# MILAB-IIT-CV/ATDN_vSLAM

Hardware: AMD Instinct MI355X
Metric: frame-pairs/sec, KITTI 1241x376 odometry inference at 1/2/4/8 MI355X (higher is better)
Workload: dtype f32 via 3xf16 split MFMA (fp32 accumulate); 1 GPU; KITTI seq-03-shaped 376x1241 uint8 frames (resident in HBM) resized to 376x1232, GMA flow 12 GRU iters + CLVO head -> 6-DoF trajectory (BASELINE configs[1]); streams_per_gpu=2, gru_iters=12, parallelism=pairs sharded x1, one all-gather of 512-d features, replicated LSTM scan

## Files before the change

atdn_vslam_amd/csrc/attention.hip:

```cpp
#include "attention.h"

#include <type_traits>

#include "conv_mfma.h"
#include "sf.h"

namespace atdn {
namespace {

constexpr float LOG2E = 1.4426950408889634f;

typedef float v4f __attribute__((ext_vector_type(4)));
typedef float f32x4v __attribute__((ext_vector_type(4)));

__device__ __forceinline__ f16x8 ld_frag(const char* p) { return *reinterpret_cast<const f16x8*>(p); }
__device__ __forceinline__ f16x8 ld_frag_nt(const char* p) {
  const v4f t = __builtin_nontemporal_load(reinterpret_cast<const v4f*>(p));
  return __builtin_bit_cast(f16x8, t);
}
__device__ __forceinline__ void st_frag_nt(char* p, f16x8 v) {
  __builtin_nontemporal_store(__builtin_bit_cast(v4f, v), reinterpret_cast<v4f*>(p));
}
__device__ __forceinline__ f32x16 mfma(f16x8 a, f16x8 b, f32x16 c) { return __builtin_amdgcn_mfma_f32_32x32x16_f16(a, b, c, 0, 0, 0); }
typedef __fp16 fp16x4_tr_ __attribute__((__vector_size__(4 * sizeof(__fp16))));
__device__ __forceinline__ f16x4 ld_tr4(const char* p) {
  return __builtin_bit_cast(f16x4, __builtin_amdgcn_ds_read_tr16_b64_v4f16(
                                       (__attribute__((address_space(3))) fp16x4_tr_*)(p)));
}

typedef unsigned int u32x2 __attribute__((ext_vector_type(2)));
typedef _Float16 f16x2 __attribute__((ext_vector_type(2)));
__device__ __forceinline__ void h3_encode(const float* v_in, float gsum, f16x8& hi, u32x2& bytes, bool& clamped) {
  float v[8];
#pragma unroll
  for (int i = 0; i < 8; ++i) v[i] = v_in[i];
  if (__builtin_expect(!(gsum <= 65504.f), 0)) {
    asm volatile("; h3_encode: saturated group");
#pragma unroll
    for (int i = 0; i < 8; ++i) {
      clamped |= !(v[i] <= 65504.f);
      v[i] = fminf(v[i], 65504.f);
    }
  }
  float hf[8];
#pragma unroll
  for (int i = 0; i < 8; ++i) {
    hi[i] = (_Float16)v[i];
    hf[i] = (float)hi[i];
  }
  const float mx = fmaxf(fmaxf(fmaxf(hf[0], hf[1]), fmaxf(hf[2], hf[3])), fmaxf(fmaxf(hf[4], hf[5]), fmaxf(hf[6], hf[7])));
  const unsigned ef = max(__float_as_uint(mx) >> 23, 113u);
  const float inv_unit = __uint_as_float((272u - ef) << 23);
  unsigned w0 = 0, w1 = 0;
#pragma unroll
  for (int i = 0; i < 8; ++i) {
    const float q = __builtin_fmaf(v[i] - hf[i], inv_unit, 128.f);
    if (i < 4) w0 = __builtin_amdgcn_cvt_pk_u8_f32(q, i, w0); else w1 = __builtin_amdgcn_cvt_pk_u8_f32(q, i - 4, w1);
  }
  bytes[0] = w0;
  bytes[1] = w1;
}
__device__ __forceinline__ f16x8 h3_decode_lo(f16x8 hi, u32x2 bytes) {
  typedef unsigned int u32x4 __attribute__((ext_vector_type(4)));
  const u32x4 hb = __builtin_bit_cast(u32x4, hi);
  const unsigned up = max(max(hb[0], hb[1]), max(hb[2], hb[3]));
  const unsigned lw = max(max(hb[0] & 0xFFFFu, hb[1] & 0xFFFFu), max(hb[2] & 0xFFFFu, hb[3] & 0xFFFFu));
  const unsigned e = max(max(up >> 26, lw >> 10), 1u);
  const float unit = __uint_as_float((e + 94u) << 23);
  const float off = -128.f * unit;
  f16x8 lo;
#pragma unroll
  for (int i = 0; i < 8; ++i) {
    const unsigned w = bytes[i >> 2];
    const float q = (float)((w >> (8 * (i & 3))) & 255u);
    float r = __builtin_fmaf(q, unit, off);
    asm("" : "+v"(r));
    lo[i] = (_Float16)r;
  }
  return lo;
}

template <bool STATS, bool FAST>
__global__ __launch_bounds__(256, 2) void qk_softmax_kernel(const float* __restrict__ qk, const AttnGeom g,
                                                           const float* __restrict__ rowmax_in,
                                                           float* __restrict__ rowmax_out, float* __restrict__ P,
                                                           float* __restrict__ rinv) {
  constexpr int KROW = 160;
  constexpr int KT = 64;
  constexpr int CH = KT * KROW;
  constexpr int IMG = 4 * CH;
  constexpr bool FULL = !STATS && !FAST;
  constexpr int RB = STATS ? 4 : 2;
  constexpr int SR = 16 * RB;
  constexpr int BLK = AT_BLK_BYTES;
  __shared__ __attribute__((aligned(16))) char lds[2 * IMG];

  const int tid = threadIdx.x, lane = tid & 63, wave = tid >> 6;
  const int nstrip = STATS ? (g.Npad + SR - 1) / SR : g.RT;
  const int tiles = (nstrip + 3) >> 2;
  const int id = xcd_remap(blockIdx.x, g.B * tiles);
  const int b = id / tiles, tile = id - b * tiles;
  const int strip = tile * 4 + wave;
  const bool strip_ok = strip < nstrip;
  const int n16 = lane & 15, g16 = lane >> 4;
  const char* qkb = reinterpret_cast<const char*>(qk + (long)b * g.N * 256);

  f16x8 qh[RB][4], ql[RB][4];
  int mrow[RB];
#pragma unroll
  for (int rb = 0; rb < RB; ++rb) {
    mrow[rb] = strip * SR + 16 * rb + n16;
    const char* qrow = qkb + (long)min(mrow[rb], g.N - 1) * 1024 + 16 * g16;
#pragma unroll
    for (int c = 0; c < 4; ++c) {
      qh[rb][c] = ld_frag(qrow + c * 128);
      if (FULL) ql[rb][c] = ld_frag(qrow + c * 128 + 64);
    }
  }

  const int lr = tid >> 3, ls = tid & 7;
  v4f kreg[2][4];
  auto fetch = [&](int j) __attribute__((always_inline)) {
#pragma unroll
    for (int i = 0; i < 2; ++i) {
      const int n = min(j * KT + lr + 32 * i, g.N - 1);
      const char* src = qkb + (long)n * 1024 + 512 + 16 * ls;
#pragma unroll
      for (int c = 0; c < 4; ++c) kreg[i][c] = *reinterpret_cast<const v4f*>(src + c * 128);
    }
  };
  auto stash = [&](int buf) __attribute__((always_inline)) {
#pragma unroll
    for (int i = 0; i < 2; ++i)
#pragma unroll
      for (int c = 0; c < 4; ++c)
        *reinterpret_cast<v4f*>(lds + buf * IMG + c * CH + (lr + 32 * i) * KROW + 16 * ls) = kreg[i][c];
  };

  const int NHT = (g.Q + 1) >> 1;
  float run[RB];
  float c0[RB];
#pragma unroll
  for (int rb = 0; rb < RB; ++rb) {
    c0[rb] = 0.f;
    run[rb] = STATS ? -INFINITY : 0.f;
    if (!STATS) c0[rb] = (float)AT_SHIFT - rowmax_in[(long)b * g.Npad + min(mrow[rb], g.Npad - 1)] * LOG2E;
  }
  bool clamped = false;
  char* pdst = reinterpret_cast<char*>(P) + ((long)(b * g.RT + min(strip, g.RT - 1)) * g.Q) * BLK;

  fetch(0);
  stash(0);
  __syncthreads();
  fetch(min(1, NHT - 1));
  for (int j = 0; j < NHT; ++j) {
    const char* img = lds + (j & 1) * IMG + n16 * KROW + 16 * g16;
    f32x4v acc[4][RB];
#pragma unroll
    for (int kb = 0; kb < 4; ++kb)
#pragma unroll
      for (int rb = 0; rb < RB; ++rb)
#pragma unroll
        for (int e = 0; e < 4; ++e) acc[kb][rb][e] = 0.f;
    f16x8 kh[2][4], kl[2][4];
    auto read_keys = [&](int set, int c) __attribute__((always_inline)) {
#pragma unroll
      for (int kb = 0; kb < 4; ++kb) {
        const char* kp = img + c * CH + 16 * kb * KROW;
        kh[set][kb] = ld_frag(kp);
        if (FULL) kl[set][kb] = ld_frag(kp + 64);
      }
    };
    read_keys(0, 0);
#pragma unroll
    for (int c = 0; c < 4; ++c) {
      if (c + 1 < 4) read_keys((c + 1) & 1, c + 1);
      __builtin_amdgcn_sched_barrier(0);
#pragma unroll
      for (int kb = 0; kb < 4; ++kb)
#pragma unroll
        for (int rb = 0; rb < RB; ++rb) {
          f32x4v a = acc[kb][rb];
          if (FULL) {
            a = __builtin_amdgcn_mfma_f32_16x16x32_f16(kl[c & 1][kb], qh[rb][c], a, 0, 0, 0);
            a = __builtin_amdgcn_mfma_f32_16x16x32_f16(kh[c & 1][kb], ql[rb][c], a, 0, 0, 0);
          }
          a = __builtin_amdgcn_mfma_f32_16x16x32_f16(kh[c & 1][kb], qh[rb][c], a, 0, 0, 0);
          acc[kb][rb] = a;
        }
      __builtin_amdgcn_sched_barrier(0);
    }
    stash((j + 1) & 1);
    fetch(min(j + 2, NHT - 1));
    auto epilogue = [&](auto tail_tag) __attribute__((always_inline)) {
      constexpr bool TAIL = decltype(tail_tag)::value;
#pragma unroll
      for (int cq = 0; cq < 2; ++cq) {
        const int key0 = j * KT + 32 * cq + 4 * g16;
        u32x2 bytes2[2] = {{0u, 0u}, {0u, 0u}};
#pragma unroll
        for (int rb = 0; rb < RB; ++rb) {
          if constexpr (STATS) {
#pragma unroll
            for (int i = 0; i < 8; ++i)
              if (!TAIL || key0 + (i & 3) + 16 * (i >> 2) < g.N) run[rb] = fmaxf(run[rb], acc[2 * cq + (i >> 2)][rb][i & 3]);
          } else {
            float v[8];
#pragma unroll
            for (int i = 0; i < 8; ++i) {
              const float x = __builtin_amdgcn_exp2f(fmaf(acc[2 * cq + (i >> 2)][rb][i & 3], LOG2E, c0[rb]));
              v[i] = (!TAIL || key0 + (i & 3) + 16 * (i >> 2) < g.N) ? x : 0.f;
            }
            const float gsum = ((v[0] + v[1]) + (v[2] + v[3])) + ((v[4] + v[5]) + (v[6] + v[7]));
            run[rb] += gsum;
            const int q = 2 * j + cq;
            if (strip_ok && q < g.Q) {
              char* d = pdst + (long)q * BLK;
              f16x8 hi;
              u32x2 bytes;
              h3_encode(v, gsum, hi, bytes, clamped);
              st_frag_nt(d + rb * 1024 + lane * 16, hi);
              bytes2[rb] = bytes;
            }
          }
        }
        if (!STATS && strip_ok && 2 * j + cq < g.Q) {
          typedef unsigned int u32x4s __attribute__((ext_vector_type(4)));
          const u32x4s bb = {bytes2[0][0], bytes2[0][1], bytes2[1][0], bytes2[1][1]};
          __builtin_nontemporal_store(bb, reinterpret_cast<u32x4s*>(pdst + (long)(2 * j + cq) * BLK + 2048 + lane * 16));
        }
      }
    };
    if ((j + 1) * KT > g.N) {
      asm volatile("; qk_softmax: tail tile");
      epilogue(std::true_type{});
    } else {
      epilogue(std::false_type{});
    }
    __syncthreads();
  }
  sf_report(clamped);
#pragma unroll
  for (int rb = 0; rb < RB; ++rb) {
    float r_ = run[rb];
    if (STATS) {
      r_ = fmaxf(r_, __shfl_xor(r_, 16));
      r_ = fmaxf(r_, __shfl_xor(r_, 32));
      if (g16 == 0 && strip_ok && mrow[rb] < g.Npad) rowmax_out[(long)b * g.Npad + mrow[rb]] = r_;
    } else {
      r_ += __shfl_xor(r_, 16);
      r_ += __shfl_xor(r_, 32);
      if (g16 == 0 && strip_ok) rinv[(long)b * g.Npad + mrow[rb]] = (mrow[rb] < g.N && r_ > 0.f) ? 1.0f / r_ : 0.f;
    }
  }
}

#ifdef ATDN_ATTN_STAMP
__device__ unsigned atdn_attn_stamps_dev[1024][2][8];
#define STAMP(k) do { __builtin_amdgcn_sched_barrier(0); asm volatile("s_waitcnt lgkmcnt(0)" ::: "memory"); \
    const unsigned long long t_ = __builtin_amdgcn_s_memtime(); asm volatile("s_waitcnt lgkmcnt(0)" ::: "memory"); \
    seg[k] += (unsigned)(t_ - tlast); tlast = t_; __builtin_amdgcn_sched_barrier(0); } while (0)
#else
#define STAMP(k) do {} while (0)
#endif
template <bool FAST, bool SPLIT = false>
__global__ __launch_bounds__(512, 2) void attn_v3_kernel(const float* __restrict__ P, const float* __restrict__ rinv,
                                                        const AttnGeom g, const float* __restrict__ vT,
                                                        const float* __restrict__ gamma, const float* __restrict__ mf,
                                                        float* __restrict__ out, const long sb, const int ld,
                                                        const int qsplit = 0, float* __restrict__ part = nullptr) {
  (void)vT; (void)gamma;
  constexpr int VROW = 544;
  constexpr int IMG = 32 * VROW;
  constexpr int BLK = AT_BLK_BYTES;
  constexpr int D = 3;
  constexpr int DEC2 = 14;
  __shared__ __attribute__((aligned(16))) char lds[3 * IMG];

  const int tid = threadIdx.x, lane = tid & 63, wave = tid >> 6;
  const bool setA = wave < 4;
  const int tiles = (g.RT + 7) >> 3;
  const int nsplit = SPLIT ? (g.Q + qsplit - 1) / qsplit : 1;
  const int id0 = xcd_remap(blockIdx.x, g.B * tiles * nsplit);
  const int ks = SPLIT ? id0 % nsplit : 0;
  const int id = SPLIT ? id0 / nsplit : id0;
  const int b = id / tiles, tile = id - b * tiles;
  const int strip = tile * 8 + wave;
  const bool strip_ok = strip < g.RT;
  const int n16 = lane & 15, g16 = lane >> 4;
  const int qlo = SPLIT ? ks * qsplit : 0;
  const int Q = SPLIT ? min(qsplit, g.Q - qlo) : g.Q;

  const char* pblk = reinterpret_cast<const char*>(P) + ((long)(b * g.RT + min(strip, g.RT - 1)) * g.Q + qlo) * BLK;
  typedef unsigned int u32x4s __attribute__((ext_vector_type(4)));
  f16x8 ring[D][2];
  u32x4s ringb[D];
  auto loadP = [&](int q, int slot) __attribute__((always_inline)) {
    const char* p = pblk + (long)min(q, Q - 1) * BLK;
#pragma unroll
    for (int rb = 0; rb < 2; ++rb) ring[slot][rb] = ld_frag_nt(p + rb * 1024 + lane * 16);
    ringb[slot] = __builtin_nontemporal_load(reinterpret_cast<const u32x4s*>(p + 2048 + lane * 16));
  };
  auto bytes_of = [&](int slot, int rb) __attribute__((always_inline)) { return u32x2{ringb[slot][2 * rb], ringb[slot][2 * rb + 1]}; };

  const int lr = (tid & 255) >> 5, ls = tid & 31;
  const char* vrow = reinterpret_cast<const char*>(mf + (long)b * sb) + 16 * ls;
  const unsigned vpitch = 4u * (unsigned)ld;
  const int vkey0 = qlo * 32 + lr;
  constexpr int NSTG = 4;
  v4f breg[2][NSTG];
  auto fetchB = [&](int q, int set) __attribute__((always_inline)) {
    const int k = vkey0 + min(q, Q - 1) * 32;
#pragma unroll
    for (int i = 0; i < NSTG; ++i)
      breg[set][i] = *reinterpret_cast<const v4f*>(vrow + (unsigned)min(k + 8 * i, g.N - 1) * vpitch);
  };
  const int boff = lr * VROW + 16 * ls;
  auto stashB = [&](int image, int set) __attribute__((always_inline)) {
#pragma unroll
    for (int i = 0; i < NSTG; ++i) *reinterpret_cast<v4f*>(lds + image * IMG + 8 * i * VROW + boff) = breg[set][i];
  };

  f32x4v acc[8][2];
#pragma unroll
  for (int cb = 0; cb < 8; ++cb)
#pragma unroll
    for (int rb = 0; rb < 2; ++rb)
#pragma unroll
      for (int e = 0; e < 4; ++e) acc[cb][rb][e] = 0.f;

  f16x8 vh[8], vl[8], ph[2], pl[2];
  const int foff = (4 * g16 + (n16 >> 2)) * VROW + 8 * (n16 & 3);
  auto read_frags = [&](int image) __attribute__((always_inline)) {
#pragma unroll
    for (int cb = 0; cb < 8; ++cb) {
      const char* vp = lds + image * IMG + foff + 128 * (cb >> 1) + 32 * (cb & 1);
      vh[cb] = __builtin_shufflevector(ld_tr4(vp), ld_tr4(vp + 16 * VROW), 0, 1, 2, 3, 4, 5, 6, 7);
      if (!FAST) vl[cb] = __builtin_shufflevector(ld_tr4(vp + 64), ld_tr4(vp + 64 + 16 * VROW), 0, 1, 2, 3, 4, 5, 6, 7);
    }
  };
  auto take_chunk = [&](int slot) __attribute__((always_inline)) {
#pragma unroll
    for (int rb = 0; rb < 2; ++rb) {
      ph[rb] = ring[slot][rb];
      if (!FAST) pl[rb] = h3_decode_lo(ph[rb], bytes_of(slot, rb));
    }
    if (!FAST) asm volatile("" :: "v"(pl[0]), "v"(pl[1]));
  };
  auto multiply = [&]() __attribute__((always_inline)) {
#pragma unroll
    for (int cb = 0; cb < 8; ++cb)
#pragma unroll
      for (int rb = 0; rb < 2; ++rb) {
        f32x4v c = acc[cb][rb];
        if (!FAST) {
          c = __builtin_amdgcn_mfma_f32_16x16x32_f16(vl[cb], ph[rb], c, 0, 0, 0);
          c = __builtin_amdgcn_mfma_f32_16x16x32_f16(vh[cb], pl[rb], c, 0, 0, 0);
        }
        c = __builtin_amdgcn_mfma_f32_16x16x32_f16(vh[cb], ph[rb], c, 0, 0, 0);
        acc[cb][rb] = c;
      }
  };
  auto multiply_next = [&](int next) __attribute__((always_inline)) {
    f16x8 pln[2];
    if (!FAST) {
#pragma unroll
      for (int rb = 0; rb < 2; ++rb) pln[rb] = h3_decode_lo(ring[next][rb], bytes_of(next, rb));
    }
    multiply();
    if (!FAST) {
#pragma unroll
      for (int k = 0; k < DEC2; ++k) {
        __builtin_amdgcn_sched_group_barrier(0x008, 1, 0);
        __builtin_amdgcn_sched_group_barrier(0x002, 2, 0);
      }
#pragma unroll
      for (int k = DEC2; k < 48; ++k) {
        __builtin_amdgcn_sched_group_barrier(0x008, 1, 0);
        __builtin_amdgcn_sched_group_barrier(0x002, 1, 0);
      }
    }
#pragma unroll
    for (int rb = 0; rb < 2; ++rb) {
      ph[rb] = ring[next][rb];
      if (!FAST) pl[rb] = pln[rb];
    }
  };

  constexpr int U = (D % 2) ? 2 * D : D;
#ifdef ATDN_ATTN_STAMP
  unsigned seg[8] = {0, 0, 0, 0, 0, 0, 0, 0};
  unsigned long long tlast = 0;
#endif
  const int nq = (Q + U - 1) / U * U;
  if (setA) {
    fetchB(0, 0);
    fetchB(1, 1);
#pragma unroll
    for (int c = 0; c < D; ++c) loadP(c, c);
    stashB(0, 0);
    stashB(1, 1);
    fetchB(2, 0);
    fetchB(3, 1);
    __syncthreads();
    read_frags(0);
    take_chunk(0);
    int image = 0;
#ifdef ATDN_ATTN_STAMP
    asm volatile("s_waitcnt lgkmcnt(0)" ::: "memory"); tlast = __builtin_amdgcn_s_memtime(); asm volatile("s_waitcnt lgkmcnt(0)" ::: "memory");
#endif
    for (int q0 = 0; q0 < nq; q0 += U) {
#pragma unroll
      for (int d = 0; d < U; ++d) {
        const int q = q0 + d;
        const int image1 = image == 2 ? 0 : image + 1, image2 = image1 == 2 ? 0 : image1 + 1;
        __builtin_amdgcn_sched_barrier(0);
        if (q < Q) multiply_next((d + 1) % D);
        __builtin_amdgcn_sched_barrier(0);
        STAMP(0);
        __syncthreads();
        STAMP(1);
        stashB(image2, d & 1);
        fetchB(q + 4, d & 1);
        loadP(q + D, d % D);
        STAMP(2);
        read_frags(image1);
        image = image1;
        STAMP(3);
        __syncthreads();
        STAMP(5);
      }
    }
  } else {
#pragma unroll
    for (int c = 0; c < D - 1; ++c) loadP(c, c);
    take_chunk(0);
    __syncthreads();
    int image = 0;
#ifdef ATDN_ATTN_STAMP
    asm volatile("s_waitcnt lgkmcnt(0)" ::: "memory"); tlast = __builtin_amdgcn_s_memtime(); asm volatile("s_waitcnt lgkmcnt(0)" ::: "memory");
#endif
    for (int q0 = 0; q0 < nq; q0 += U) {
#pragma unroll
      for (int d = 0; d < U; ++d) {
        const int q = q0 + d;
        loadP(q + D - 1, (d + D - 1) % D);
        STAMP(0);
        read_frags(image);
        image = image == 2 ? 0 : image + 1;
        STAMP(1);
        __syncthreads();
        STAMP(3);
        __builtin_amdgcn_sched_barrier(0);
        if (q < Q) multiply_next((d + 1) % D);
        __builtin_amdgcn_sched_barrier(0);
        STAMP(4);
        __syncthreads();
        STAMP(5);
      }
    }
  }

#ifdef ATDN_ATTN_STAMP
  if (lane == 0 && (wave == 0 || wave == 4) && blockIdx.x < 1024) {
#pragma unroll
    for (int k = 0; k < 8; ++k) atdn_attn_stamps_dev[blockIdx.x][wave >> 2][k] = seg[k];
  }
#endif
  if constexpr (SPLIT) {
    float* pp = part + ((long)ks * g.B + b) * g.Npad * 128;
#pragma unroll
    for (int rb = 0; rb < 2; ++rb) {
      const int m = strip * 32 + 16 * rb + n16;
      if (strip_ok && m < g.N) {
#pragma unroll
        for (int cb = 0; cb < 8; ++cb)
          *reinterpret_cast<float4*>(pp + (long)m * 128 + 16 * cb + 4 * g16) =
              make_float4(acc[cb][rb][0], acc[cb][rb][1], acc[cb][rb][2], acc[cb][rb][3]);
      }
    }
    return;
  }
  float* ob = out + (long)b * sb;
  bool clamped = false;
#pragma unroll
  for (int rb = 0; rb < 2; ++rb) {
    const int m = strip * 32 + 16 * rb + n16;
    if (strip_ok && m < g.N) {
      const float rv = rinv[(long)b * g.Npad + m];
#pragma unroll
      for (int cb = 0; cb < 8; ++cb) {
        const int c = 16 * cb + 4 * g16;
        const float4 o = make_float4(rv * acc[cb][rb][0], rv * acc[cb][rb][1], rv * acc[cb][rb][2], rv * acc[cb][rb][3]);
        sf_store4_flag(ob, (long)m * ld, c, o, clamped);
      }
    }
  }
  sf_report(clamped);
}

__global__ __launch_bounds__(256) void attn_reduce_kernel(const float* __restrict__ part, const int nsplit, const AttnGeom g,
                                                          const float* __restrict__ rinv, const float* __restrict__ gamma,
                                                          const float* __restrict__ mf, float* __restrict__ out, const long sb,
                                                          const int ld) {
  const long i = (long)blockIdx.x * 256 + threadIdx.x;
  const long rows = (long)g.B * g.N;
  bool clamped = false;
  if (i < rows * 32) {
    const long row = i >> 5;
    const int c = (int)(i & 31) * 4;
    const int b = (int)(row / g.N), m = (int)(row - (long)b * g.N);
    const long slab = (long)g.B * g.Npad * 128;
    const float* p = part + ((long)b * g.Npad + m) * 128 + c;
    float4 s = *reinterpret_cast<const float4*>(p);
    for (int k = 1; k < nsplit; ++k) {
      const float4 t = *reinterpret_cast<const float4*>(p + k * slab);
      s.x += t.x; s.y += t.y; s.z += t.z; s.w += t.w;
    }
    const float rv = rinv[(long)b * g.Npad + m];
    sf_store4_flag(out + (long)b * sb, (long)m * ld, c, make_float4(rv * s.x, rv * s.y, rv * s.z, rv * s.w), clamped);
  }
  sf_report(clamped);
}

__global__ __launch_bounds__(64) void attn_decode_kernel(const float* __restrict__ P, const float* __restrict__ rinv,
                                                         const AttnGeom g, float* __restrict__ rows) {
  const long blk = blockIdx.x;
  const int q = (int)(blk % g.Q);
  const long bs = blk / g.Q;
  const int strip = (int)(bs % g.RT), b = (int)(bs / g.RT);
  const int lane = threadIdx.x, n = lane & 15, gq = lane >> 4;
  const char* p = reinterpret_cast<const char*>(P) + blk * AT_BLK_BYTES;
#pragma unroll
  for (int rb = 0; rb < 2; ++rb) {
    const int m = strip * 32 + 16 * rb + n;
    if (m >= g.N) continue;
    const float rv = rinv[(long)b * g.Npad + m];
    float* row = rows + ((long)b * g.N + m) * g.ldN + q * 32;
    const f16x8 hi = ld_frag(p + rb * 1024 + lane * 16);
    const f16x8 lo = h3_decode_lo(hi, *reinterpret_cast<const u32x2*>(p + 2048 + lane * 16 + rb * 8));
#pragma unroll
    for (int i = 0; i < 8; ++i) row[4 * gq + (i & 3) + 16 * (i >> 2)] = ((float)hi[i] + (float)lo[i]) * rv;
  }
}

}

#ifdef ATDN_ATTN_STAMP
extern "C" int atdn_attn_stamps(unsigned* out) {
  return (int)hipMemcpyFromSymbol(out, HIP_SYMBOL(atdn_attn_stamps_dev), sizeof(unsigned) * 1024 * 2 * 8);
}
#endif

void launch_qk_rowmax(const float* qk, const AttnGeom& g, float* rowmax, hipStream_t st) {
  const int nblk = g.B * (((g.Npad + 63) / 64 + 3) / 4);
  hipLaunchKernelGGL((qk_softmax_kernel<true, false>), dim3(nblk), dim3(256), 0, st, qk, g, nullptr, rowmax, nullptr, nullptr);
  ATDN_HIP(hipGetLastError());
}

void launch_qk_softmax(const float* qk, const AttnGeom& g, const float* rowmax, float* P, float* rinv, bool fast,
                       hipStream_t st) {
  const int nblk = g.B * ((g.RT + 3) / 4);
  const dim3 gr(nblk), bl(256);
  if (fast) hipLaunchKernelGGL((qk_softmax_kernel<false, true>), gr, bl, 0, st, qk, g, rowmax, nullptr, P, rinv);
  else hipLaunchKernelGGL((qk_softmax_kernel<false, false>), gr, bl, 0, st, qk, g, rowmax, nullptr, P, rinv);
  ATDN_HIP(hipGetLastError());
}

int attn_v_splits(const AttnGeom& g) {
  const int tiles = g.B * ((g.RT + 7) / 8);
  int n = std::min(8, std::max(1, 256 / std::max(tiles, 1)));
  while (n > 1 && (g.Q + n - 1) / n < 8) --n;
  return n;
}

void launch_attn_v(const float* P, const float* rinv, const AttnGeom& g, const float* vT, const float* gamma,
                   const float* mf, float* out, long sb, int ld, bool fast, hipStream_t st, float* part) {
  ATDN_CHECK(g.ldN % 32 == 0 && g.Q * 32 == g.ldN && ld % 32 == 0, "attention geometry");
  const int want = !part ? 1 : attn_v_splits(g);
  if (want > 1) {
    const int qsplit = (g.Q + want - 1) / want, nsplit = (g.Q + qsplit - 1) / qsplit;
    const dim3 gr(g.B * ((g.RT + 7) / 8) * nsplit), bl(512);
    if (fast) hipLaunchKernelGGL((attn_v3_kernel<true, true>), gr, bl, 0, st, P, rinv, g, vT, gamma, mf, out, sb, ld, qsplit, part);
    else hipLaunchKernelGGL((attn_v3_kernel<false, true>), gr, bl, 0, st, P, rinv, g, vT, gamma, mf, out, sb, ld, qsplit, part);
    ATDN_HIP(hipGetLastError());
    const long n4 = (long)g.B * g.N * 32;
    hipLaunchKernelGGL(attn_reduce_kernel, dim3((unsigned)((n4 + 255) / 256)), dim3(256), 0, st, part, nsplit, g, rinv, gamma, mf, out, sb, ld);
    ATDN_HIP(hipGetLastError());
    return;
  }
  const dim3 gr(g.B * ((g.RT + 7) / 8)), bl(512);
  if (fast) hipLaunchKernelGGL((attn_v3_kernel<true>), gr, bl, 0, st, P, rinv, g, vT, gamma, mf, out, sb, ld);
  else hipLaunchKernelGGL((attn_v3_kernel<false>), gr, bl, 0, st, P, rinv, g, vT, gamma, mf, out, sb, ld);
  ATDN_HIP(hipGetLastError());
}

void launch_attn_decode(const float* P, const float* rinv, const AttnGeom& g, float* rows, hipStream_t st) {
  const long nblk = (long)g.B * g.RT * g.Q;
  hipLaunchKernelGGL(attn_decode_kernel, dim3((unsigned)nblk), dim3(64), 0, st, P, rinv, g, rows);
  ATDN_HIP(hipGetLastError());
}

}
```

Measured before the change: 437.0 frame-pairs/s.

## Stage attention V tiles directly into LDS with global_load_lds and re-pair layout

Replaces the register-staged V fetch plus LDS store (fetchB/stashB) with direct global-to-LDS dwordx4 loads issued via inline asm with m0, changing the LDS image layout to key-pairs per wave with swizzled source columns. Explicit vmcnt waits replace the implicit register dependency, and the prefetch distance shrinks from q+4 to q+2. The MFMA/decode interleave schedule is also reshaped with a leading head of MFMAs. This aims to free VGPRs and remove VALU/LDS-store work from the loop, at the risk of subtle layout or wait-count errors.

New measurement: 438.3 frame-pairs/s (median of 6 runs). Within noise of the previous version (+0.3%).

```diff
diff --git a/atdn_vslam_amd/csrc/attention.hip b/atdn_vslam_amd/csrc/attention.hip
--- a/atdn_vslam_amd/csrc/attention.hip
+++ b/atdn_vslam_amd/csrc/attention.hip
@@ -270,11 +270,12 @@
                                                         float* __restrict__ out, const long sb, const int ld,
                                                         const int qsplit = 0, float* __restrict__ part = nullptr) {
   (void)vT; (void)gamma;
-  constexpr int VROW = 544;
-  constexpr int IMG = 32 * VROW;
+  constexpr int VPAIR = 1088;
+  constexpr int IMG = 16 * VPAIR;
   constexpr int BLK = AT_BLK_BYTES;
   constexpr int D = 3;
-  constexpr int DEC2 = 14;
+  constexpr int HEAD = 12;
+  constexpr int NP = FAST ? 2 : 3;
   __shared__ __attribute__((aligned(16))) char lds[3 * IMG];
 
   const int tid = threadIdx.x, lane = tid & 63, wave = tid >> 6;
@@ -293,32 +294,36 @@
 
   const char* pblk = reinterpret_cast<const char*>(P) + ((long)(b * g.RT + min(strip, g.RT - 1)) * g.Q + qlo) * BLK;
   typedef unsigned int u32x4s __attribute__((ext_vector_type(4)));
+  unsigned plane = 16u * lane;
   f16x8 ring[D][2];
   u32x4s ringb[D];
   auto loadP = [&](int q, int slot) __attribute__((always_inline)) {
-    const char* p = pblk + (long)min(q, Q - 1) * BLK;
-#pragma unroll
-    for (int rb = 0; rb < 2; ++rb) ring[slot][rb] = ld_frag_nt(p + rb * 1024 + lane * 16);
-    ringb[slot] = __builtin_nontemporal_load(reinterpret_cast<const u32x4s*>(p + 2048 + lane * 16));
+    const char* p = pblk + (long)min(q, Q - 1) * BLK + plane;
+#pragma unroll
+    for (int rb = 0; rb < 2; ++rb) ring[slot][rb] = ld_frag_nt(p + rb * 1024);
+    ringb[slot] = __builtin_nontemporal_load(reinterpret_cast<const u32x4s*>(p + 2048));
   };
   auto bytes_of = [&](int slot, int rb) __attribute__((always_inline)) { return u32x2{ringb[slot][2 * rb], ringb[slot][2 * rb + 1]}; };
 
-  const int lr = (tid & 255) >> 5, ls = tid & 31;
-  const char* vrow = reinterpret_cast<const char*>(mf + (long)b * sb) + 16 * ls;
+  const int ls = tid & 31, podd = lane >> 5;
+  const char* vsrc = reinterpret_cast<const char*>(mf + (long)b * sb) + 16 * ((ls - 2 * podd) & 31);
   const unsigned vpitch = 4u * (unsigned)ld;
-  const int vkey0 = qlo * 32 + lr;
+  const int vkey0 = qlo * 32 + 2 * (wave & 3) + podd;
+  const unsigned vdst0 = (unsigned)(unsigned long)(__attribute__((address_space(3))) char*)lds +
+                         (unsigned)(__builtin_amdgcn_readfirstlane(wave) & 3) * VPAIR;
   constexpr int NSTG = 4;
-  v4f breg[2][NSTG];
-  auto fetchB = [&](int q, int set) __attribute__((always_inline)) {
+  auto stageV = [&](int q, int image) __attribute__((always_inline)) {
     const int k = vkey0 + min(q, Q - 1) * 32;
 #pragma unroll
-    for (int i = 0; i < NSTG; ++i)
-      breg[set][i] = *reinterpret_cast<const v4f*>(vrow + (unsigned)min(k + 8 * i, g.N - 1) * vpitch);
-  };
-  const int boff = lr * VROW + 16 * ls;
-  auto stashB = [&](int image, int set) __attribute__((always_inline)) {
-#pragma unroll
-    for (int i = 0; i < NSTG; ++i) *reinterpret_cast<v4f*>(lds + image * IMG + 8 * i * VROW + boff) = breg[set][i];
+    for (int i = 0; i < NSTG; ++i) {
+      const char* src = vsrc + (unsigned)min(k + 8 * i, g.N - 1) * vpitch;
+      const unsigned dst = vdst0 + (unsigned)(image * IMG + 4 * i * VPAIR);
+      unsigned keep;
+      asm volatile("s_mov_b32 %0, m0\n\ts_mov_b32 m0, %2\n\ts_nop 0\n\tglobal_load_lds_dwordx4 %1, off\n\ts_mov_b32 m0, %0"
+                   : "=&s"(keep) : "v"(src), "s"(dst) : "memory");
+    }
+    asm volatile("" : "+v"(plane));
+    __builtin_amdgcn_sched_barrier(0);
   };
 
   f32x4v acc[8][2];
@@ -330,13 +335,17 @@
       for (int e = 0; e < 4; ++e) acc[cb][rb][e] = 0.f;
 
   f16x8 vh[8], vl[8], ph[2], pl[2];
-  const int foff = (4 * g16 + (n16 >> 2)) * VROW + 8 * (n16 & 3);
+  const int fkey = 4 * g16 + (n16 >> 2);
+  const int foff = (fkey >> 1) * VPAIR + (fkey & 1) * 544 + 8 * (n16 & 3);
+  const int foffw = foff - 512 * (fkey & 1);
   auto read_frags = [&](int image) __attribute__((always_inline)) {
 #pragma unroll
     for (int cb = 0; cb < 8; ++cb) {
-      const char* vp = lds + image * IMG + foff + 128 * (cb >> 1) + 32 * (cb & 1);
-      vh[cb] = __builtin_shufflevector(ld_tr4(vp), ld_tr4(vp + 16 * VROW), 0, 1, 2, 3, 4, 5, 6, 7);
-      if (!FAST) vl[cb] = __builtin_shufflevector(ld_tr4(vp + 64), ld_tr4(vp + 64 + 16 * VROW), 0, 1, 2, 3, 4, 5, 6, 7);
+      const int kc = 128 * (cb >> 1) + 32 * (cb & 1);
+      const char* vp = lds + image * IMG + foff + kc;
+      vh[cb] = __builtin_shufflevector(ld_tr4(vp), ld_tr4(vp + 8 * VPAIR), 0, 1, 2, 3, 4, 5, 6, 7);
+      const char* vq = lds + image * IMG + (kc + 64 == 480 ? foffw : foff) + kc + 64;
+      if (!FAST) vl[cb] = __builtin_shufflevector(ld_tr4(vq), ld_tr4(vq + 8 * VPAIR), 0, 1, 2, 3, 4, 5, 6, 7);
     }
   };
   auto take_chunk = [&](int slot) __attribute__((always_inline)) {
@@ -369,15 +378,18 @@
     }
     multiply();
     if (!FAST) {
+      constexpr int DEC2 = 62 - (48 - HEAD);
+      static_assert(DEC2 >= 0 && DEC2 <= 48 - HEAD, "the decode must fit behind the head at two instructions per gap");
+      __builtin_amdgcn_sched_group_barrier(0x008, HEAD, 0);
 #pragma unroll
       for (int k = 0; k < DEC2; ++k) {
+        __builtin_amdgcn_sched_group_barrier(0x002, 2, 0);
         __builtin_amdgcn_sched_group_barrier(0x008, 1, 0);
-        __builtin_amdgcn_sched_group_barrier(0x002, 2, 0);
-      }
-#pragma unroll
-      for (int k = DEC2; k < 48; ++k) {
+      }
+#pragma unroll
+      for (int k = DEC2; k < 48 - HEAD; ++k) {
+        __builtin_amdgcn_sched_group_barrier(0x002, 1, 0);
         __builtin_amdgcn_sched_group_barrier(0x008, 1, 0);
-        __builtin_amdgcn_sched_group_barrier(0x002, 1, 0);
       }
     }
 #pragma unroll
@@ -394,14 +406,11 @@
 #endif
   const int nq = (Q + U - 1) / U * U;
   if (setA) {
-    fetchB(0, 0);
-    fetchB(1, 1);
+    stageV(0, 0);
+    stageV(1, 1);
 #pragma unroll
     for (int c = 0; c < D; ++c) loadP(c, c);
-    stashB(0, 0);
-    stashB(1, 1);
-    fetchB(2, 0);
-    fetchB(3, 1);
+    asm volatile("s_waitcnt vmcnt(0)" ::: "memory");
     __syncthreads();
     read_frags(0);
     take_chunk(0);
@@ -417,12 +426,13 @@
         __builtin_amdgcn_sched_barrier(0);
         if (q < Q) multiply_next((d + 1) % D);
         __builtin_amdgcn_sched_barrier(0);
+        asm volatile("s_waitcnt vmcnt(%0)" :: "n"(NP) : "memory");
         STAMP(0);
         __syncthreads();
         STAMP(1);
-        stashB(image2, d & 1);
-        fetchB(q + 4, d & 1);
+        stageV(q + 2, image2);
         loadP(q + D, d % D);
+        __builtin_amdgcn_sched_barrier(0);
         STAMP(2);
         read_frags(image1);
         image = image1;
@@ -431,6 +441,7 @@
         STAMP(5);
       }
     }
+    asm volatile("s_waitcnt vmcnt(0)" ::: "memory");
   } else {
 #pragma unroll
     for (int c = 0; c < D - 1; ++c) loadP(c, c);
```
